# SCUT-CCNL/3DSIFT

Measured on AMD Instinct MI355X. Metric: Mvoxels/s end-to-end KpSiftAlgorithm on 512^3 fp32, higher is better.
Workload: dtype f32

## Files before the change

### 3dsift_amd/capi.py

```python
import ctypes as C
import os

import numpy as np

HERE = os.path.dirname(os.path.abspath(__file__))
LIB_PATH = os.environ.get("S3D_LIB") or os.path.join(HERE, "libsift3d_hip.so")
DESC = 768

KP_DTYPE = np.dtype(
    [
        ("x", "<f4"), ("y", "<f4"), ("z", "<f4"),
        ("scale", "<f4"),
        ("octave", "<i4"), ("level", "<i4"),
        ("rx", "<f4"), ("ry", "<f4"), ("rz", "<f4"),
        ("win", "<f4", (3,)),
        ("eigvalue", "<f4", (3,)),
        ("eigvector", "<f4", (9,)),
        ("Rotation", "<f4", (9,)),
        ("str_tensor", "<f4", (9,)),
    ]
)
assert KP_DTYPE.itemsize == 168

SYMBOLS = [
# ... 5 lines not shown
    "sift3d_match_handles",
    "sift3d_default_detect_options", "sift3d_set_detect_options", "sift3d_get_detect_options", "sift3d_get_refined",
    "sift3d_default_ransac_options", "sift3d_fit_affine", "sift3d_fit_affine_local",
    "sift3d_default_icgn_options", "sift3d_icgn_init_from_fits", "sift3d_icgn",
    "sift3d_device_count", "sift3d_error_string", "sift3d_last_error",
    "sift3d_slab_min_halo", "sift3d_slab_arena_floats", "sift3d_slab_create", "sift3d_slab_buffer", "sift3d_slab_upload",
    "sift3d_slab_input_absmax", "sift3d_slab_input_scale", "sift3d_slab_level", "sift3d_slab_level_hw", "sift3d_slab_halo_planes",
    "sift3d_slab_sync", "sift3d_slab_get_dogmax", "sift3d_slab_set_dogmax", "sift3d_slab_detect", "sift3d_slab_describe",
    "sift3d_slab_decimate", "sift3d_slab_admits", "sift3d_slab_set_ghost", "sift3d_slab_min_halo_ghost", "sift3d_create_seeded", "sift3d_seed_upload", "sift3d_set_describe_partition",
    "sift3d_export_device", "sift3d_import_descriptors_device", "sift3d_run_partial_orientation",
    "sift3d_export_orientation_device", "sift3d_import_orientation_device", "sift3d_run_describe",
    "sift3d_set_stream", "sift3d_slab_export_dogmax_device", "sift3d_slab_import_dogmax_device", "sift3d_slab_decimate_async",
    "sift3d_slab_set_desc_partial", "sift3d_slab_min_halo_partial", "sift3d_slab_record_bytes", "sift3d_slab_desc_reach", "sift3d_slab_orient",
    "sift3d_slab_export_records", "sift3d_slab_describe_partial", "sift3d_slab_describe_finish", "sift3d_slab_orient_launch",
    "sift3d_slab_orient_count",
    "sift3d_slab_keypoints_launch", "sift3d_slab_keypoints_count", "sift3d_slab_describe_finish_launch", "sift3d_slab_describe_finish_count",
    "sift3d_seed_buffer", "sift3d_sharded_plan", "sift3d_slab_describe_launch", "sift3d_sharded_traffic",
    "sift3d_sharded_create", "sift3d_sharded_create_ex", "sift3d_sharded_run", "sift3d_sharded_num_keypoints", "sift3d_sharded_get_keypoints", "sift3d_sharded_info",
    "sift3d_sharded_error", "sift3d_sharded_destroy",
    "sift3d_test_hook", "sift3d_debug_counters", "sift3d_debug_face_lookup", "sift3d_match_times", "sift3d_debug_copy_bandwidth",
    "sift3d_match_warmup", "sift3d_test_staging_slice", "sift3d_test_slab_plan", "sift3d_test_sharded_time_rank",
]
HOOKS = {"dog_eager": 0, "glast_eager": 1, "det_serial": 2, "separable": 3, "desc_nocache": 4, "match_nodma": 5, "one_stream": 6,
         "desc_mass_shift": 7, "list_cap": 8, "peer_copy": 9, "desc_nosplit": 10, "march_tiles": 11, "desc_exact_cells": 12, "lazy_generic": 13, "sharded_fail_rank": 14}
ORIENT_WORDS = 34
SHARDED_PARTIAL_WINDOWS = 1
SHARDED_WHOLE_WINDOWS = 2
SHARDED_COPY_TRANSPORT = 4
SHARDED_GHOST_OCTAVE0 = 8


class Params(C.Structure):
    _fields_ = [("num_kp_levels", C.c_int), ("sigma_default", C.c_float), ("sigma_n_default", C.c_float),
                ("peak_thresh", C.c_float), ("max_eig_thres", C.c_float), ("corner_thresh", C.c_float)]


class DetectOptions(C.Structure):
    _fields_ = [("neighbours", C.c_int), ("refine", C.c_int), ("max_offset", C.c_float), ("contrast_thresh", C.c_float),
                ("edge_ratio", C.c_float), ("reserved", C.c_int * 3)]


assert C.sizeof(DetectOptions) == 32

REFINED_DTYPE = np.dtype([("rx", "<f4"), ("ry", "<f4"), ("rz", "<f4"), ("scale", "<f4"), ("offset", "<f4", (4,)), ("contrast", "<f4")])
assert REFINED_DTYPE.itemsize == 36


# ... 919 lines not shown
```

### 3dsift_amd/csrc/context.hip

```cpp
#include <float.h>
#include <math.h>
#include <stdlib.h>
#include <string.h>

#include <algorithm>
#include <atomic>
#include <mutex>
#include <thread>

#include "ctx_internal.h"

#pragma clang fp contract(off)

namespace s3d {

static thread_local std::string g_last_error;
void set_last_error(const std::string &s) { g_last_error = s; }

int set_device(int device) {
	int n = 0;
	if (hipGetDeviceCount(&n) != hipSuccess || n <= 0) {
		set_last_error("no HIP device visible: this library has no CPU fallback");
		return SIFT3D_ERR_NO_DEVICE;
	}
// ... 25 lines not shown
	S3D_HIP(hipMalloc(&c->d_kpout, sizeof(sift3d_keypoint) * (size_t)c->kp_cap));
	S3D_HIP(hipMalloc(&c->d_desc, sizeof(float) * kDesc * (size_t)c->kp_cap));
	S3D_HIP(hipMalloc(&c->d_xyz, sizeof(float) * 3 * (size_t)c->kp_cap));
	{
		const unsigned scap = 4096;
		const size_t words = (size_t)scap * (kDesc + 8 + 1);
		int *base = nullptr;
		S3D_HIP(hipMalloc(&base, sizeof(int) * words));
		hipError_t me = hipMemsetAsync(base, 0, sizeof(int) * words, c->stream);
		if (me == hipSuccess) me = hipStreamSynchronize(c->stream);
		if (me != hipSuccess) {
			hipFree(base);
			set_last_error(std::string("HIP error: ") + hipGetErrorString(me) + " (clearing the split-window scratch)");
			return SIFT3D_ERR_HIP;
		}
		c->dsplit.gacc = base;
		c->dsplit.gmass = reinterpret_cast<float *>(base + (size_t)scap * kDesc);
		c->dsplit.gdone = reinterpret_cast<unsigned *>(base + (size_t)scap * (kDesc + 8));
		c->dsplit.cap = scap;
	}
	S3D_HIP(hipMalloc(&c->d_prov, sizeof(unsigned) * ((size_t)c->ext_cap + 1)));
	c->det.prov = c->d_prov; c->det.prov_count = c->d_prov + c->ext_cap; c->det.prov_cap = c->ext_cap;
	if (c->det_o.size() > 1) {
		const size_t n2 = c->det_o.size() - 1;
		const unsigned slice = std::max(64u, (unsigned)(c->ext_cap / n2));
		S3D_HIP(hipMalloc(&c->d_prov2, sizeof(unsigned) * ((size_t)slice + 1) * n2));
		for (size_t o = 1; o < c->det_o.size(); o++) {
			c->det_o[o].prov = c->d_prov2 + (o - 1) * ((size_t)slice + 1);
			c->det_o[o].prov_count = c->det_o[o].prov + slice;
			c->det_o[o].prov_cap = slice;
		}
	}
	return SIFT3D_OK;
}

extern "C" void sift3d_default_params(sift3d_params *p) {
	if (!p) return;
	p->num_kp_levels = 3;
	p->sigma_default = 1.6f;
	p->sigma_n_default = 1.15f;
	p->peak_thresh = 0.1f;
	p->max_eig_thres = 0.9f;
	p->corner_thresh = 0.4f;
}

extern "C" void sift3d_default_detect_options(sift3d_detect_options *o) {
	if (!o) return;
	memset(o, 0, sizeof(*o));
	o->neighbours = 8;
	o->refine = 0;
	o->max_offset = 0.5f;
	o->contrast_thresh = 0.0f;
// ... 525 lines not shown
		DetectOpts dopt;
		dopt.neighbours = c->dopt.neighbours; dopt.refine = c->dopt.refine;
		dopt.max_offset = c->dopt.max_offset; dopt.contrast_thresh = c->dopt.contrast_thresh; dopt.edge_ratio = c->dopt.edge_ratio;
		const DetectOpts *dop = c->run_full ? &dopt : nullptr;
		if (upto >= 3)
			for (int o = 0; o < c->noct; o++) {
				DetectLevels &DL = DLs[(size_t)o];
				memset(&DL, 0, sizeof(DL));
				for (int i = 1; i <= nl; i++) {
					DL.cur[i - 1] = c->dog[(size_t)o * c->nd + i].d;
					DL.prev[i - 1] = c->dog[(size_t)o * c->nd + i - 1].d;
					DL.next[i - 1] = c->dog[(size_t)o * c->nd + i + 1].d;
					DL.absmax_bits[i - 1] = c->d_dogmax + (size_t)o * c->nd + i;
					DL.level_id[i - 1] = i;
					DL.scale[i - 1] = c->dog[(size_t)o * c->nd + i].scale;
				}
				if (c->dog_elide) {
					DL.prev0_hi = c->gss[(size_t)o * c->ng + 1].d; DL.prev0_lo = c->gss[(size_t)o * c->ng].d;
					DL.nextl_hi = c->gss[(size_t)o * c->ng + c->nd].d; DL.nextl_lo = c->gss[(size_t)o * c->ng + c->nd - 1].d;
					DL.nextl_slot = nl - 1;
					if (c->g_last_elide) { DL.nextl_hi = nullptr; DL.lazy_src = DL.nextl_lo; }
				}
			}
		hipStream_t sb = two ? c->ostream[1] : st;
		if (early) {
			const Level &C0 = c->dog[(size_t)0 * c->nd + 1];
			S3D_HIP(hipEventRecord(c->ev_det_fork, st));
			launch_detect_mark(DLs[0], nl, C0.nx, C0.ny, C0.zr_all(), c->p.peak_thresh, 0 + c->octave_base, c->det, st, lt, dop);
			S3D_HIP(hipStreamWaitEvent(sb, c->ev_det_fork, 0));
			for (int o = 1; o < c->noct; o++) S3D_HIP(hipStreamWaitEvent(sb, c->ev_done[o], 0));
			S3D_HIP(hipEventRecord(c->ev[1], sb));
			S3D_HIP(hipEventRecord(c->ev[2], sb));
		} else {
			for (int o = 1; o < c->noct; o++) S3D_HIP(hipStreamWaitEvent(st, c->ev_done[o], 0));
			S3D_HIP(hipEventRecord(c->ev[1], st));
			S3D_HIP(hipEventRecord(c->ev[2], st));
		}
		if (upto >= 3) {
			if (two && !early) { S3D_HIP(hipEventRecord(c->ev_det_fork, st)); S3D_HIP(hipStreamWaitEvent(sb, c->ev_det_fork, 0)); }
			if (two) {
				hipStream_t sc = (c->noct > 2 && c->ostream.size() > 2 && c->ostream[2] != st && c->ostream[2] != sb) ? c->ostream[2] : sb;
				const bool own = early && sc != sb;
				if (sc != sb && !own) { S3D_HIP(hipEventRecord(c->ev_det_fork2, sb)); S3D_HIP(hipStreamWaitEvent(sc, c->ev_det_fork2, 0)); }
				for (int o = 1; o < c->noct; o++) {
					const Level &C = c->dog[(size_t)o * c->nd + 1];
					if (own && o >= 2) S3D_HIP(hipStreamWaitEvent(sc, c->ev_done[o], 0));
					launch_detect_mark(DLs[(size_t)o], nl, C.nx, C.ny, C.zr_all(), c->p.peak_thresh, o + c->octave_base, c->det_o[(size_t)o], o == 1 ? sb : sc, lt, dop);
				}
				S3D_HIP(hipEventRecord(c->ev_det_join, sb));
				if (sc != sb) { S3D_HIP(hipEventRecord(c->ev_det_join2, sc)); S3D_HIP(hipStreamWaitEvent(sb, c->ev_det_join2, 0)); S3D_HIP(hipEventRecord(c->ev_det_join, sb)); }
			}
			std::vector<DetectEmitItem> rest;
			for (int o = 0; o < c->noct; o++) {
				const Level &C = c->dog[(size_t)o * c->nd + 1];
				const DetectBufs &b = (two && o > 0) ? c->det_o[(size_t)o] : c->det;
				if (!(two && o > 0) && !(early && o == 0)) launch_detect_mark(DLs[(size_t)o], nl, C.nx, C.ny, C.zr_all(), c->p.peak_thresh, o + c->octave_base, b, st, lt, dop);
				if (two && o == 1) S3D_HIP(hipStreamWaitEvent(st, c->ev_det_join, 0));
				if (two && o > 0 && c->noct - 1 <= 8) rest.push_back(DetectEmitItem{&DLs[(size_t)o], nl, C.nx, C.ny, C.zr_all(), o + c->octave_base, &b});
				else launch_detect_emit(DLs[(size_t)o], nl, C.nx, C.ny, C.zr_all(), o + c->octave_base, b, c->d_ext, c->ext_cap, st);
			}
			if (!rest.empty()) launch_detect_emit_multi(rest.data(), (int)rest.size(), c->d_ext, c->ext_cap, c->d_total, st);
		}
		S3D_HIP(hipEventRecord(c->ev[3], st));
		if (upto >= 4) {
			launch_orient(c->d_ext, c->d_codes, c->d_total, c->ext_cap, c->d_levels, c->d_luts, c->d_lutpool, c->p.max_eig_thres,
			              c->p.corner_thresh, part_orient ? c->part_rank : 0, part_orient ? c->part_world : 1, c->d_order, c->d_nkp + 3, st);
			launch_slots(c->d_ext, c->d_codes, c->d_total, c->ext_cap, c->d_nkp, c->d_order, c->kp_cap, c->d_slots_part, st);
		}
		S3D_HIP(hipEventRecord(c->ev[4], st));
		if (upto >= 5) {
			launch_describe(c->d_ext, c->d_total, c->ext_cap, c->d_levels, c->d_luts, c->d_lutpool, c->d_desc, c->kp_cap, c->part_rank,
			                c->part_world, c->d_order, c->d_nkp, c->d_nkp + 1, st, c->desc_lut_lds, &c->dsplit);
		}
		if (upto >= 4) launch_finalize(c->d_ext, c->d_total, c->ext_cap, upto >= 5, c->d_kpout, c->d_xyz, c->kp_cap, st);
		if (upto >= 4 && c->run_refine) {
			DogTable T;
			memset(&T, 0, sizeof(T));
			T.octave_base = c->octave_base;
			for (int o = 0; o < c->noct && o < kDogTabOct; o++) {
				const Level &D0 = c->dog[(size_t)o * c->nd];
				T.nx[o] = D0.nx; T.ny[o] = D0.ny;
// ... 308 lines not shown
```

### 3dsift_amd/csrc/kernels_detect.hip

```cpp
#include <stdio.h>
#include <string.h>
#include <stdlib.h>

#include <algorithm>

#include "sift3d_internal.h"

namespace s3d {

#ifndef S3D_DET_ROWS
#define S3D_DET_ROWS 32
#endif
#ifndef S3D_DET_QUEUE
#define S3D_DET_QUEUE 640
#endif
#ifndef S3D_DETDIAG
#define S3D_DETDIAG 0
#endif
#ifndef S3D_DET_LEAN
#define S3D_DET_LEAN 1
#endif
#ifndef S3D_DET_XPRE
#define S3D_DET_XPRE 0
#endif
constexpr int kRows = S3D_DET_ROWS;
constexpr int kThreads = 256;

constexpr int kQueue = S3D_DET_QUEUE;
__global__ void __launch_bounds__(kThreads) k_mark(DetectLevels L, int nx, int ny, ZRange zr, int nyb, float peak_thresh,
                                                   unsigned long long *__restrict__ masks, unsigned *__restrict__ block_counts,
                                                   unsigned *__restrict__ prov, unsigned *__restrict__ prov_count, unsigned prov_cap,
                                                   unsigned *__restrict__ total) {
	__shared__ unsigned s_cnt[kThreads / 64];
	__shared__ uint2 s_q[kThreads / 64][kQueue];
	extern __shared__ unsigned long long s_mask_dyn[];
	const int segw = min((nx + 63) >> 6, 64);
	const int b = blockIdx.x;
	const int nz = zr.zo1 - zr.zo0;
	const int yb = b % nyb, zi = (b / nyb) % nz, lvl = b / (nyb * nz);
	const int z = zr.zo0 + zi;
	const int zg = z + zr.zoff;
	const float *__restrict__ cur = L.cur[lvl];
	const float *__restrict__ prev = L.prev[lvl];
	const float *__restrict__ next = L.next[lvl];
	const bool lazy_prev = lvl == 0 && L.prev0_hi != nullptr, lazy_next = lvl == L.nextl_slot && L.nextl_hi != nullptr;
	const bool lazy_g = lvl == L.nextl_slot && L.lazy_src != nullptr;
	const float thr = peak_thresh * __uint_as_float(*L.absmax_bits[lvl]);
	const int wpr = (nx + 63) >> 6;
	const int lane = threadIdx.x & 63, wid = threadIdx.x >> 6;
	const size_t sy = (size_t)nx, sz = (size_t)nx * ny;
	const bool z_in = (zg >= 1 && zg <= zr.nzg - 2);
	const int y0 = yb * kRows;
	constexpr int kBatch = 8;
	const int nrows = min(kRows, ny - y0);
	const int swid = __builtin_amdgcn_readfirstlane(wid);
	const int r_lo = swid * (kRows / 4), r_hi = min(nrows, (swid + 1) * (kRows / 4));
	uint2 *q = s_q[swid];
	unsigned long long *mloc = s_mask_dyn + (size_t)swid * (kRows / 4) * segw;
	for (int i = lane; i < (kRows / 4) * segw; i += 64) mloc[i] = 0ull;
	const unsigned long long lt = (1ull << lane) - 1ull;
// ... 139 lines not shown
					evaluate(qn, 64, seg0);
				}
			}
		}
		if (qn > 0) evaluate(0, qn, seg0);
		qn = 0;
		for (int ry = r_lo; ry < r_hi; ry++) {
			unsigned long long *mrow = masks + ((size_t)(lvl * nz + zi) * ny + (y0 + ry)) * wpr;
			for (int xw = seg0 + lane; xw < seg1; xw += 64) {
				const unsigned long long m = mloc[(ry - r_lo) * segw + xw - seg0];
				mrow[xw] = m;
				cnt += (unsigned)__popcll(m);
				mloc[(ry - r_lo) * segw + xw - seg0] = 0ull;
			}
		}
	}
#pragma unroll
	for (int o = 32; o > 0; o >>= 1) cnt += __shfl_xor(cnt, o, 64);
	if (lane == 0) s_cnt[wid] = cnt;
	__syncthreads();
	if (threadIdx.x == 0) block_counts[b] = s_cnt[0] + s_cnt[1] + s_cnt[2] + s_cnt[3];
}

__device__ __forceinline__ void lazy_tap_src(int p, int d, int n, int &lo, int &hi, float &frac, bool interior) {
	if (interior) { lo = hi = p - d; frac = 0.0f; return; }
	const int dim_end = n - 1;
	float c = (float)p - (float)d * 1.0f;
	if (c < 0.0f) c = -1.0f * c;
	else if (c >= (float)dim_end) c = (float)(2 * dim_end) - c - 0.1f;
	lo = (int)c;
	frac = c - (float)lo;
	hi = lo + 1;
	lo = min(max(lo, 0), dim_end);
	hi = min(max(hi, 0), dim_end);
}
static_assert(kLazySlots / 2 - 1 == 25, "k_lazy_next's wide instantiation covers kLazySlots");
constexpr int kLwN = 17, kLwPieces = kLwN * kLwN * 5, kLwInstr = (kLwPieces + 63) / 64, kLwFloats = kLwInstr * 256, kLwWaves = 2;
__global__ void __launch_bounds__(64 * kLwWaves) k_lazy_wave(DetectLevels L, Taps t, int nx, int ny, ZRange zr, int nyb,
                                                            const unsigned *__restrict__ prov, const unsigned *__restrict__ prov_count,
                                                            unsigned prov_cap, unsigned long long *__restrict__ masks,
                                                            unsigned *__restrict__ block_counts) {
	__shared__ __attribute__((aligned(1024))) float s_buf[kLwWaves][kLwFloats];
	constexpr int H = 8, N = kLwN;
	const int lane = threadIdx.x & 63, wid = __builtin_amdgcn_readfirstlane((int)(threadIdx.x >> 6));
	float *blk = s_buf[wid];
	const unsigned lds_base = (unsigned)(size_t)blk;
	const unsigned count = min(*prov_count, prov_cap);
	const int lvl = L.nextl_slot;
	const float *__restrict__ src = L.lazy_src;
	const float *__restrict__ cur = L.cur[lvl];
	const int wpr = (nx + 63) >> 6, nzs = zr.zo1 - zr.zo0, nzg = zr.nzg;
	const size_t sy = (size_t)nx, sz = (size_t)nx * ny;
	unsigned voff[kLwInstr];
#pragma unroll
	for (int j = 0; j < kLwInstr; j++) {
		const int p = min(64 * j + lane, kLwPieces - 1), row = p / 5, q = p - 5 * row, zi = row / N, yi = row - zi * N;
		voff[j] = (unsigned)(((size_t)zi * sz + (size_t)yi * sy + (size_t)(4 * q)) * sizeof(float));
	}
	const unsigned nwaves = gridDim.x * kLwWaves;
	for (unsigned e = blockIdx.x * kLwWaves + (unsigned)wid; e < count; e += nwaves) {
		const unsigned ent = prov[e];
		const size_t ic = (size_t)(ent & 0x7FFFFFFFu);
		const bool as_max = (ent >> 31) != 0;
		const int zl = (int)(ic / sz), rem = (int)(ic - (size_t)zl * sz), y = rem / nx, x = rem - y * nx;
		const int zg = zl + zr.zoff;
		if (!(x >= H && x <= nx - 2 - H && y >= H && y <= ny - 2 - H && zg >= H && zg <= nzg - 2 - H)) continue;
		const int shift = min(max(0, x + 11 - (nx - 1)), x - H);
		const float *base = src + ic - (size_t)H * sz - (size_t)H * sy - (size_t)(H + shift);
#pragma unroll
		for (int j = 0; j < kLwInstr; j++) {
			unsigned keep;
			asm volatile("s_mov_b32 %0, m0\n\ts_mov_b32 m0, %3\n\ts_nop 0\n\tglobal_load_lds_dwordx4 %1, %2\n\ts_mov_b32 m0, %0"
			             : "=&s"(keep) : "v"(voff[j]), "s"(base), "s"(lds_base + 1024u * (unsigned)j) : "memory");
		}
		const float centre = src[ic], v = cur[ic];
		asm volatile("s_waitcnt vmcnt(0)" ::: "memory");
		__builtin_amdgcn_wave_barrier();
#pragma unroll
		for (int rq = 0; rq < (N * N + 63) / 64; rq++) {
			const int row = min(lane + 64 * rq, N * N - 1);
			const float *r = blk + row * 20 + shift;
			float acc = 0.0f;
#pragma unroll
// ... 12 lines not shown
			__builtin_amdgcn_fence(__ATOMIC_RELEASE, "wavefront");
			__builtin_amdgcn_wave_barrier();
			if (lane < N) blk[pl * N * 20] = acc;
		}
		__builtin_amdgcn_fence(__ATOMIC_RELEASE, "wavefront");
		__builtin_amdgcn_wave_barrier();
		__builtin_amdgcn_fence(__ATOMIC_ACQUIRE, "wavefront");
		{
			float acc = 0.0f;
#pragma unroll
			for (int k = 0; k < N; k++) acc = acc + t.w[k] * blk[(2 * H - k) * N * 20];
			const float n7 = (acc - centre) * (-1.0f);
			if (lane == 0 && (as_max ? (v > n7) : (v < n7))) {
				const int zi = zl - zr.zo0;
				atomicOr(&masks[((size_t)(lvl * nzs + zi) * ny + y) * wpr + (x >> 6)], 1ull << (x & 63));
				atomicAdd(&block_counts[(lvl * nzs + zi) * nyb + y / kRows], 1u);
			}
		}
		__builtin_amdgcn_fence(__ATOMIC_RELEASE, "wavefront");
		__builtin_amdgcn_wave_barrier();
	}
}

template <int kLT>
__global__ void __launch_bounds__(256) k_lazy_next(DetectLevels L, Taps t, int nx, int ny, ZRange zr, int nyb,
                                                   const unsigned *__restrict__ prov, const unsigned *__restrict__ prov_count,
                                                   unsigned prov_cap, unsigned long long *__restrict__ masks,
                                                   unsigned *__restrict__ block_counts, int skip_interior) {
	constexpr int kLR = kLT + 1;
	constexpr int kLP = kLR + 1;
	__shared__ float s_blk[kLR * kLR * kLP];
	__shared__ float s_x[kLR * kLR];
	__shared__ float s_y[kLR];
	__shared__ float s_w[kMaxTaps];
	__shared__ int s_lo[3][kLT], s_hi[3][kLT];
	__shared__ float s_fr[3][kLT];
	__shared__ int s_rng[6];
	const int hw = t.hw, nt = 2 * hw + 1, tid = threadIdx.x;
	for (int i = tid; i < nt; i += 256) s_w[i] = t.w[i];
	const unsigned count = min(*prov_count, prov_cap);
	const int lvl = L.nextl_slot;
	const float *__restrict__ src = L.lazy_src;
	const float *__restrict__ cur = L.cur[lvl];
	const int wpr = (nx + 63) >> 6, nzs = zr.zo1 - zr.zo0, nzg = zr.nzg;
	const size_t sy = (size_t)nx, sz = (size_t)nx * ny;
	__shared__ unsigned s_list[256];
	__shared__ unsigned s_nlist;
	for (unsigned e0 = blockIdx.x; e0 < count; e0 += 256 * gridDim.x) {
	__syncthreads();
	if (tid == 0) s_nlist = 0u;
	__syncthreads();
	if (e0 + (unsigned)tid * gridDim.x < count) {
		const unsigned ent = prov[e0 + (unsigned)tid * gridDim.x];
		const size_t ic = (size_t)(ent & 0x7FFFFFFFu);
		const int zl = (int)(ic / sz), rem = (int)(ic - (size_t)zl * sz), y = rem / nx, x = rem - y * nx;
		const int zg = zl + zr.zoff;
		const bool inner = x >= hw && x <= nx - 2 - hw && y >= hw && y <= ny - 2 - hw && zg >= hw && zg <= nzg - 2 - hw;
		if (!(skip_interior && inner)) s_list[atomicAdd(&s_nlist, 1u)] = ent;
	}
	__syncthreads();
	const unsigned nlist = s_nlist;
	for (unsigned li = 0; li < nlist; li++) {
		const unsigned ent = s_list[li];
		const size_t ic = (size_t)(ent & 0x7FFFFFFFu);
		const bool as_max = (ent >> 31) != 0;
		const int zl = (int)(ic / sz), rem = (int)(ic - (size_t)zl * sz), y = rem / nx, x = rem - y * nx;
		const int zg = zl + zr.zoff;
		const bool ix = x >= hw && x <= nx - 2 - hw, iy = y >= hw && y <= ny - 2 - hw, iz = zg >= hw && zg <= nzg - 2 - hw;
		__syncthreads();
		if (tid < 3 * nt) {
			const int ax = tid / nt, k = tid - ax * nt;
			int lo, hi; float fr;
			if (ax == 0) lazy_tap_src(x, k - hw, nx, lo, hi, fr, ix);
			else if (ax == 1) lazy_tap_src(y, k - hw, ny, lo, hi, fr, iy);
			else lazy_tap_src(zg, k - hw, nzg, lo, hi, fr, iz);
			s_lo[ax][k] = lo; s_hi[ax][k] = hi; s_fr[ax][k] = fr;
// ... 56 lines not shown
		if (tid == 0) {
			const float *pl = s_y - zmin;
			float acc = 0.0f;
			if (iz) {
				for (int k = 0; k < nt; k++) acc = acc + s_w[k] * pl[s_lo[2][k]];
			} else {
				for (int k = 0; k < nt; k++) {
					const float f = s_fr[2][k];
					acc = acc + s_w[k] * ((1.0f - f) * pl[s_lo[2][k]] + f * pl[s_hi[2][k]]);
				}
			}
			const float n7 = (acc - src[ic]) * (-1.0f);
			const float v = cur[ic];
			if (as_max ? (v > n7) : (v < n7)) {
				const int zi = zl - zr.zo0;
				atomicOr(&masks[((size_t)(lvl * nzs + zi) * ny + y) * wpr + (x >> 6)], 1ull << (x & 63));
				atomicAdd(&block_counts[(lvl * nzs + zi) * nyb + y / kRows], 1u);
			}
		}
	}
	}
}

__device__ __forceinline__ unsigned scan_octave(const unsigned *__restrict__ block_counts, unsigned *__restrict__ block_offsets, unsigned nblocks,
                                                unsigned base, unsigned *s_wave) {
	const unsigned t = threadIdx.x;
	const unsigned chunk = (((nblocks + 1023u) / 1024u) + 3u) & ~3u;
	const unsigned lo = min(t * chunk, nblocks), hi = min(lo + chunk, nblocks);
	const bool vec = (((size_t)block_counts | (size_t)block_offsets) & 15) == 0 && hi - lo == chunk && chunk <= 32;
	unsigned cnt[32];
	unsigned sum = 0;
	if (vec) {
#pragma unroll
		for (unsigned q = 0; q < 8; q++)
			if (q * 4 < chunk) {
				const uint4 c4 = *reinterpret_cast<const uint4 *>(block_counts + lo + 4 * q);
				cnt[4 * q] = c4.x; cnt[4 * q + 1] = c4.y; cnt[4 * q + 2] = c4.z; cnt[4 * q + 3] = c4.w;
				sum += c4.x + c4.y + c4.z + c4.w;
			}
	} else {
		for (unsigned i = lo; i < hi; i++) sum += block_counts[i];
	}
	unsigned v = sum;
	const int lane = t & 63, wid = t >> 6;
#pragma unroll
	for (int o = 1; o < 64; o <<= 1) {
// ... 25 lines not shown
	__syncthreads();
	const unsigned nbase = s_wave[0];
	__syncthreads();
	return nbase;
}

__global__ void __launch_bounds__(1024) k_scan(const unsigned *__restrict__ block_counts, unsigned *__restrict__ block_offsets,
                                               unsigned nblocks, unsigned *__restrict__ total) {
	__shared__ unsigned s_wave[16];
	const unsigned nb = scan_octave(block_counts, block_offsets, nblocks, total[0], s_wave);
	if (threadIdx.x == 0) total[0] = nb;
}

struct EmitOct {
	const unsigned long long *masks;
	const unsigned *counts;
	unsigned *offsets;
	int nx, ny, nyb, octave;
	ZRange zr;
	unsigned nblocks, block0;
	int level_id[kMaxKpLevels];
	float scale[kMaxKpLevels];
};
struct EmitMulti { EmitOct o[8]; int n; };
__global__ void __launch_bounds__(1024) k_scan_multi(EmitMulti M, unsigned *__restrict__ total) {
	__shared__ unsigned s_wave[16];
	unsigned base = total[0];
	__syncthreads();
	for (int k = 0; k < M.n; k++) base = scan_octave(M.o[k].counts, M.o[k].offsets, M.o[k].nblocks, base, s_wave);
	if (threadIdx.x == 0) total[0] = base;
}

__device__ __forceinline__ void emit_block(int b, const unsigned long long *__restrict__ masks, const unsigned *__restrict__ block_offsets, int nx,
                                           int ny, const ZRange &zr, int nyb, int octave, const int *level_id, const float *scale,
                                           DevKp *__restrict__ out, unsigned cap, unsigned *__restrict__ total, unsigned *s_wave) {
	const int nz = zr.zo1 - zr.zo0;
	const int yb = b % nyb, zi = (b / nyb) % nz, lvl = b / (nyb * nz);
	const int z = zr.zo0 + zi + zr.zoff;
	const int wpr = (nx + 63) >> 6;
	const int y0 = yb * kRows;
	const int nwords = min(kRows, ny - y0) * wpr;
	const int lane = threadIdx.x & 63, wid = threadIdx.x >> 6;
	unsigned running = block_offsets[b];
	for (int w0 = 0; w0 < nwords; w0 += kThreads) {
		const int wi = w0 + threadIdx.x;
		unsigned long long m = 0;
		int y = 0, xw = 0;
// ... 34 lines not shown
			}
			pos++;
		}
		running += all;
	}
}

__global__ void __launch_bounds__(kThreads) k_emit(const unsigned long long *__restrict__ masks,
                                                   const unsigned *__restrict__ block_offsets, int nx, int ny, ZRange zr, int nyb,
                                                   int octave, DetectLevels L, DevKp *__restrict__ out, unsigned cap,
                                                   unsigned *__restrict__ total) {
	__shared__ unsigned s_wave[kThreads / 64];
	emit_block((int)blockIdx.x, masks, block_offsets, nx, ny, zr, nyb, octave, L.level_id, L.scale, out, cap, total, s_wave);
}

__global__ void __launch_bounds__(kThreads) k_emit_multi(EmitMulti M, DevKp *__restrict__ out, unsigned cap, unsigned *__restrict__ total) {
	__shared__ unsigned s_wave[kThreads / 64];
	int k = 0;
	while (k + 1 < M.n && blockIdx.x >= M.o[k + 1].block0) k++;
	const EmitOct &E = M.o[k];
	emit_block((int)(blockIdx.x - E.block0), E.masks, E.offsets, E.nx, E.ny, E.zr, E.nyb, E.octave, E.level_id, E.scale, out, cap, total, s_wave);
}

void launch_detect_mark(const DetectLevels &L, int nlevels, int nx, int ny, const ZRange &zr, float peak_thresh, int octave,
                        const DetectBufs &b, hipStream_t st, const Taps *lazy_taps, const DetectOpts *opt) {
	if (opt) { launch_mark_full(L, nlevels, nx, ny, zr, kRows, peak_thresh, *opt, b, st); return; }
	const int nyb = (ny + kRows - 1) / kRows;
	const int nzl = zr.zo1 - zr.zo0;
	if (nzl <= 0) return;
	const unsigned nblocks = (unsigned)(nlevels * nzl * nyb);
	if (nblocks == 0) return;
	const bool lazy = L.lazy_src != nullptr && lazy_taps != nullptr && b.prov != nullptr;
	if (lazy) (void)hipMemsetAsync(b.prov_count, 0, sizeof(unsigned), st);
	const size_t mask_lds = sizeof(unsigned long long) * (kThreads / 64) * (kRows / 4) * (size_t)std::min((nx + 63) >> 6, 64);
	hipLaunchKernelGGL(k_mark, dim3(nblocks), dim3(kThreads), mask_lds, st, L, nx, ny, zr, nyb, peak_thresh, b.masks, b.block_counts, b.prov,
	                   b.prov_count, b.prov_cap, b.total);
	if (lazy) {
		const bool wave_form = lazy_taps->hw == 8 && !hook(SIFT3D_HOOK_LAZY_GENERIC) && (size_t)nx * (size_t)ny * 17u * sizeof(float) < ((size_t)1 << 32);
		if (wave_form)
			hipLaunchKernelGGL(k_lazy_wave, dim3(256 * 3), dim3(64 * kLwWaves), 0, st, L, *lazy_taps, nx, ny, zr, nyb, b.prov, b.prov_count, b.prov_cap,
			                   b.masks, b.block_counts);
		if (2 * lazy_taps->hw + 1 <= 17)
			hipLaunchKernelGGL(k_lazy_next<17>, dim3(wave_form ? 1536 : 1024), dim3(256), 0, st, L, *lazy_taps, nx, ny, zr, nyb, b.prov, b.prov_count, b.prov_cap,
			                   b.masks, b.block_counts, wave_form ? 1 : 0);
		else
			hipLaunchKernelGGL(k_lazy_next<25>, dim3(512), dim3(256), 0, st, L, *lazy_taps, nx, ny, zr, nyb, b.prov, b.prov_count, b.prov_cap,
			                   b.masks, b.block_counts, 0);
	}
}

void launch_detect_emit(const DetectLevels &L, int nlevels, int nx, int ny, const ZRange &zr, int octave, const DetectBufs &b, DevKp *out,
                        unsigned cap, hipStream_t st) {
	const int nyb = (ny + kRows - 1) / kRows;
	const int nzl = zr.zo1 - zr.zo0;
	if (nzl <= 0) return;
	const unsigned nblocks = (unsigned)(nlevels * nzl * nyb);
	if (nblocks == 0) return;
	hipLaunchKernelGGL(k_scan, dim3(1), dim3(1024), 0, st, b.block_counts, b.block_offsets, nblocks, b.total);
	hipLaunchKernelGGL(k_emit, dim3(nblocks), dim3(kThreads), 0, st, b.masks, b.block_offsets, nx, ny, zr, nyb, octave, L, out, cap,
	                   b.total);
}

void launch_detect_emit_multi(const DetectEmitItem *items, int n, DevKp *out, unsigned cap, unsigned *total, hipStream_t st) {
	EmitMulti M;
	memset(&M, 0, sizeof(M));
	unsigned blocks = 0;
	for (int k = 0; k < n && M.n < 8; k++) {
		const DetectEmitItem &it = items[k];
		const int nyb = (it.ny + kRows - 1) / kRows, nzl = it.zr.zo1 - it.zr.zo0;
		if (nzl <= 0) continue;
		const unsigned nblocks = (unsigned)(it.nlevels * nzl * nyb);
		if (nblocks == 0) continue;
		EmitOct &E = M.o[M.n++];
		E.masks = it.b->masks; E.counts = it.b->block_counts; E.offsets = it.b->block_offsets;
		E.nx = it.nx; E.ny = it.ny; E.nyb = nyb; E.octave = it.octave; E.zr = it.zr; E.nblocks = nblocks; E.block0 = blocks;
		for (int l = 0; l < kMaxKpLevels; l++) { E.level_id[l] = it.L->level_id[l]; E.scale[l] = it.L->scale[l]; }
		blocks += nblocks;
	}
	if (M.n == 0) return;
	hipLaunchKernelGGL(k_scan_multi, dim3(1), dim3(1024), 0, st, M, total);
	hipLaunchKernelGGL(k_emit_multi, dim3(blocks), dim3(kThreads), 0, st, M, out, cap, total);
}

void launch_detect_octave(const DetectLevels &L, int nlevels, int nx, int ny, const ZRange &zr, float peak_thresh, int octave,
                          const DetectBufs &b, DevKp *out, unsigned cap, hipStream_t st, const Taps *lazy_taps) {
	launch_detect_mark(L, nlevels, nx, ny, zr, peak_thresh, octave, b, st, lazy_taps);
	launch_detect_emit(L, nlevels, nx, ny, zr, octave, b, out, cap, st);
}

void preload_detect_kernels() { hipFuncAttributes a; (void)hipFuncGetAttributes(&a, reinterpret_cast<const void *>(&k_scan)); }
// ... 3 lines not shown
```

### 3dsift_amd/csrc/sift3d_internal.h

```cpp
#pragma once

#include <hip/hip_runtime.h>
#include <stdint.h>

#include <string>
#include <vector>

#include "../../include/sift3d_hip.h"
#include "../../include/sift3d_hip_test.h"

#pragma clang fp contract(off)

namespace s3d {

#ifndef S3D_MAX_HW
#define S3D_MAX_HW 64
#endif
constexpr int kMaxHW = S3D_MAX_HW;
constexpr int kMaxTaps = 2 * kMaxHW + 1;
constexpr int kDesc = SIFT3D_DESC_NUMEL;
constexpr int kFaces = 20;

struct Taps {
	int hw;
// ... 115 lines not shown
	const unsigned *absmax_bits[kMaxKpLevels];
	int level_id[kMaxKpLevels];
	float scale[kMaxKpLevels];
};
constexpr int kLazySlots = 52;
struct DetectOpts {
	int neighbours = 8, refine = 0;
	float max_offset = 0.5f, contrast_thresh = 0.0f, edge_ratio = 0.0f;
};
void launch_detect_mark(const DetectLevels &L, int nlevels, int nx, int ny, const ZRange &zr, float peak_thresh, int octave,
                        const DetectBufs &b, hipStream_t st, const Taps *lazy_taps, const DetectOpts *opt = nullptr);
void launch_mark_full(const DetectLevels &L, int nlevels, int nx, int ny, const ZRange &zr, int rows, float peak_thresh, const DetectOpts &opt,
                      const DetectBufs &b, hipStream_t st);
constexpr int kDogTabOct = 12, kDogTabLv = 8;
struct DogTable {
	const float *d[kDogTabOct][kDogTabLv];
	int nx[kDogTabOct], ny[kDogTabOct];
	int octave_base;
};
void launch_detect_emit(const DetectLevels &L, int nlevels, int nx, int ny, const ZRange &zr, int octave, const DetectBufs &b, DevKp *out,
                        unsigned cap, hipStream_t st);
struct DetectEmitItem { const DetectLevels *L; int nlevels, nx, ny; ZRange zr; int octave; const DetectBufs *b; };
void launch_detect_emit_multi(const DetectEmitItem *items, int n, DevKp *out, unsigned cap, unsigned *total, hipStream_t st);
void launch_detect_octave(const DetectLevels &L, int nlevels, int nx, int ny, const ZRange &zr, float peak_thresh, int octave,
                          const DetectBufs &b, DevKp *out, unsigned cap, hipStream_t st, const Taps *lazy_taps = nullptr);

#ifdef __HIPCC__
typedef const float __attribute__((address_space(1))) *gfloat_p;
__device__ __forceinline__ gfloat_p as_global(const float *p) { return (gfloat_p)p; }
#endif

struct LevelRef {
	const float *d;
	int nx, ny, nz;
	float unit;
	int zoff;
};
void launch_orient(DevKp *kps, int *codes, const unsigned *d_count, unsigned cap, const LevelRef *d_levels ,
                   const WinLut *d_luts, const float *d_lutpool, float max_eig, float corner, int part_rank, int part_world,
                   int *redo_list , unsigned *redo_count,
                   hipStream_t st);
constexpr int kOrientWords = 34;
void launch_orient_pack(const DevKp *kps, const unsigned *d_count, unsigned cap, int *dst, int part_rank, int part_world, hipStream_t st);
void launch_orient_unpack(DevKp *kps, int *codes, const unsigned *d_count, unsigned cap, const int *src, hipStream_t st);
size_t slots_scratch_words();
void launch_slots(DevKp *kps, const int *codes, const unsigned *d_count, unsigned cap, unsigned *d_nkp, int *order, unsigned kp_cap,
// ... 89 lines not shown
```

Measured before the change: 19410.

## Batch small-octave detect marking and lazy refinement into multi-octave launches

Octaves 2 and up, which are small, no longer get separate mark and lazy-refinement launches. They are grouped into one table-driven k_mark launch plus combined lazy wave and next launches, with the grids split by each octave's voxel share. The prov_count counters are packed contiguously so one memset clears them all. Octave 0 is also folded into the multi-octave emit pass. The aim is to cut kernel launch and memset overhead on tiny grids, at the cost of a larger kernel-argument struct and a per-block search through the table.

```diff
diff --git a/3dsift_amd/capi.py b/3dsift_amd/capi.py
--- a/3dsift_amd/capi.py
+++ b/3dsift_amd/capi.py
@@ -51,7 +51,8 @@
     "sift3d_match_warmup", "sift3d_test_staging_slice", "sift3d_test_slab_plan", "sift3d_test_sharded_time_rank",
 ]
 HOOKS = {"dog_eager": 0, "glast_eager": 1, "det_serial": 2, "separable": 3, "desc_nocache": 4, "match_nodma": 5, "one_stream": 6,
-         "desc_mass_shift": 7, "list_cap": 8, "peer_copy": 9, "desc_nosplit": 10, "march_tiles": 11, "desc_exact_cells": 12, "lazy_generic": 13, "sharded_fail_rank": 14}
+         "desc_mass_shift": 7, "list_cap": 8, "peer_copy": 9, "desc_nosplit": 10, "march_tiles": 11, "desc_exact_cells": 12, "lazy_generic": 13, "sharded_fail_rank": 14,
+         "det_unbatched": 15}
 ORIENT_WORDS = 34
 SHARDED_PARTIAL_WINDOWS = 1
 SHARDED_WHOLE_WINDOWS = 2
diff --git a/3dsift_amd/csrc/context.hip b/3dsift_amd/csrc/context.hip
--- a/3dsift_amd/csrc/context.hip
+++ b/3dsift_amd/csrc/context.hip
@@ -71,12 +71,12 @@
 	S3D_HIP(hipMalloc(&c->d_prov, sizeof(unsigned) * ((size_t)c->ext_cap + 1)));
 	c->det.prov = c->d_prov; c->det.prov_count = c->d_prov + c->ext_cap; c->det.prov_cap = c->ext_cap;
 	if (c->det_o.size() > 1) {
-		const size_t n2 = c->det_o.size() - 1;
+		const size_t n2 = c->det_o.size() - 1, head = (n2 + 63) & ~(size_t)63;
 		const unsigned slice = std::max(64u, (unsigned)(c->ext_cap / n2));
-		S3D_HIP(hipMalloc(&c->d_prov2, sizeof(unsigned) * ((size_t)slice + 1) * n2));
+		S3D_HIP(hipMalloc(&c->d_prov2, sizeof(unsigned) * (head + (size_t)slice * n2)));
 		for (size_t o = 1; o < c->det_o.size(); o++) {
-			c->det_o[o].prov = c->d_prov2 + (o - 1) * ((size_t)slice + 1);
-			c->det_o[o].prov_count = c->det_o[o].prov + slice;
+			c->det_o[o].prov = c->d_prov2 + head + (o - 1) * (size_t)slice;
+			c->det_o[o].prov_count = c->d_prov2 + (o - 1);
 			c->det_o[o].prov_cap = slice;
 		}
 	}
@@ -648,11 +648,20 @@
 					if (c->g_last_elide) { DL.nextl_hi = nullptr; DL.lazy_src = DL.nextl_lo; }
 				}
 			}
+		const bool tables_fit = c->noct - 1 <= 8 && !hook(SIFT3D_HOOK_DET_UNBATCHED);
+		static const int det_batch_mode = dev_tune_i("S3D_DET_BATCH", 1), emit_one_mode = dev_tune_i("S3D_EMIT_ONE", 1);
+		const bool batch = two && tables_fit && !dop && det_batch_mode != 0 && c->noct - 2 <= detect_mark_multi_max();
+		const bool emit_one = tables_fit && emit_one_mode != 0;
+		static const int lazy_all_mode = dev_tune_i("S3D_LAZY_ALL", 0);
+		const bool lazy_all = batch && early && lt != nullptr && lazy_all_mode != 0 && c->noct <= detect_mark_multi_max();
 		hipStream_t sb = two ? c->ostream[1] : st;
 		if (early) {
 			const Level &C0 = c->dog[(size_t)0 * c->nd + 1];
 			S3D_HIP(hipEventRecord(c->ev_det_fork, st));
-			launch_detect_mark(DLs[0], nl, C0.nx, C0.ny, C0.zr_all(), c->p.peak_thresh, 0 + c->octave_base, c->det, st, lt, dop);
+			if (lazy_all) {
+				const DetectEmitItem i0{&DLs[0], nl, C0.nx, C0.ny, C0.zr_all(), 0 + c->octave_base, &c->det};
+				launch_detect_mark_multi(&i0, 1, c->p.peak_thresh, st, lt, 1);
+			} else launch_detect_mark(DLs[0], nl, C0.nx, C0.ny, C0.zr_all(), c->p.peak_thresh, 0 + c->octave_base, c->det, st, lt, dop);
 			S3D_HIP(hipStreamWaitEvent(sb, c->ev_det_fork, 0));
 			for (int o = 1; o < c->noct; o++) S3D_HIP(hipStreamWaitEvent(sb, c->ev_done[o], 0));
 			S3D_HIP(hipEventRecord(c->ev[1], sb));
@@ -668,11 +677,17 @@
 				hipStream_t sc = (c->noct > 2 && c->ostream.size() > 2 && c->ostream[2] != st && c->ostream[2] != sb) ? c->ostream[2] : sb;
 				const bool own = early && sc != sb;
 				if (sc != sb && !own) { S3D_HIP(hipEventRecord(c->ev_det_fork2, sb)); S3D_HIP(hipStreamWaitEvent(sc, c->ev_det_fork2, 0)); }
+				std::vector<DetectEmitItem> small;
 				for (int o = 1; o < c->noct; o++) {
 					const Level &C = c->dog[(size_t)o * c->nd + 1];
 					if (own && o >= 2) S3D_HIP(hipStreamWaitEvent(sc, c->ev_done[o], 0));
-					launch_detect_mark(DLs[(size_t)o], nl, C.nx, C.ny, C.zr_all(), c->p.peak_thresh, o + c->octave_base, c->det_o[(size_t)o], o == 1 ? sb : sc, lt, dop);
+					if (batch && o >= 2) small.push_back(DetectEmitItem{&DLs[(size_t)o], nl, C.nx, C.ny, C.zr_all(), o + c->octave_base, &c->det_o[(size_t)o]});
+					else if (lazy_all) {
+						const DetectEmitItem i1{&DLs[(size_t)o], nl, C.nx, C.ny, C.zr_all(), o + c->octave_base, &c->det_o[(size_t)o]};
+						launch_detect_mark_multi(&i1, 1, c->p.peak_thresh, sb, lt, 1);
+					} else launch_detect_mark(DLs[(size_t)o], nl, C.nx, C.ny, C.zr_all(), c->p.peak_thresh, o + c->octave_base, c->det_o[(size_t)o], o == 1 ? sb : sc, lt, dop);
 				}
+				if (!small.empty()) launch_detect_mark_multi(small.data(), (int)small.size(), c->p.peak_thresh, sc, lt, lazy_all ? 1 : 3);
 				S3D_HIP(hipEventRecord(c->ev_det_join, sb));
 				if (sc != sb) { S3D_HIP(hipEventRecord(c->ev_det_join2, sc)); S3D_HIP(hipStreamWaitEvent(sb, c->ev_det_join2, 0)); S3D_HIP(hipEventRecord(c->ev_det_join, sb)); }
 			}
@@ -682,7 +697,15 @@
 				const DetectBufs &b = (two && o > 0) ? c->det_o[(size_t)o] : c->det;
 				if (!(two && o > 0) && !(early && o == 0)) launch_detect_mark(DLs[(size_t)o], nl, C.nx, C.ny, C.zr_all(), c->p.peak_thresh, o + c->octave_base, b, st, lt, dop);
 				if (two && o == 1) S3D_HIP(hipStreamWaitEvent(st, c->ev_det_join, 0));
-				if (two && o > 0 && c->noct - 1 <= 8) rest.push_back(DetectEmitItem{&DLs[(size_t)o], nl, C.nx, C.ny, C.zr_all(), o + c->octave_base, &b});
+				if (lazy_all && o == 1) {
+					std::vector<DetectEmitItem> all;
+					for (int q = 0; q < c->noct; q++) {
+						const Level &Cq = c->dog[(size_t)q * c->nd + 1];
+						all.push_back(DetectEmitItem{&DLs[(size_t)q], nl, Cq.nx, Cq.ny, Cq.zr_all(), q + c->octave_base, q ? &c->det_o[(size_t)q] : &c->det});
+					}
+					launch_detect_mark_multi(all.data(), (int)all.size(), c->p.peak_thresh, st, lt, 2);
+				}
+				if (two && (o > 0 || emit_one) && tables_fit) rest.push_back(DetectEmitItem{&DLs[(size_t)o], nl, C.nx, C.ny, C.zr_all(), o + c->octave_base, &b});
 				else launch_detect_emit(DLs[(size_t)o], nl, C.nx, C.ny, C.zr_all(), o + c->octave_base, b, c->d_ext, c->ext_cap, st);
 			}
 			if (!rest.empty()) launch_detect_emit_multi(rest.data(), (int)rest.size(), c->d_ext, c->ext_cap, c->d_total, st);
diff --git a/3dsift_amd/csrc/kernels_detect.hip b/3dsift_amd/csrc/kernels_detect.hip
--- a/3dsift_amd/csrc/kernels_detect.hip
+++ b/3dsift_amd/csrc/kernels_detect.hip
@@ -27,15 +27,37 @@
 constexpr int kThreads = 256;
 
 constexpr int kQueue = S3D_DET_QUEUE;
-__global__ void __launch_bounds__(kThreads) k_mark(DetectLevels L, int nx, int ny, ZRange zr, int nyb, float peak_thresh,
-                                                   unsigned long long *__restrict__ masks, unsigned *__restrict__ block_counts,
-                                                   unsigned *__restrict__ prov, unsigned *__restrict__ prov_count, unsigned prov_cap,
-                                                   unsigned *__restrict__ total) {
+constexpr int kMarkMax = 8;
+struct MarkOct {
+	DetectLevels L;
+	int nx, ny, nyb, skip_interior;
+	ZRange zr;
+	unsigned long long *masks;
+	unsigned *block_counts, *prov, *prov_count, *total;
+	unsigned prov_cap;
+	unsigned block0;
+	unsigned wave0, wave_n;
+	unsigned next0, next_n;
+};
+template <int kN> struct MarkTable { MarkOct o[kN]; int n; };
+typedef MarkTable<kMarkMax> MarkMulti;
+
+template <int kN>
+__global__ void __launch_bounds__(kThreads) k_mark(MarkTable<kN> M, float peak_thresh) {
+	int k = 0;
+	if (kN > 1) while (k + 1 < M.n && blockIdx.x >= M.o[k + 1].block0) k++;
+	const MarkOct &E = M.o[k];
+	const DetectLevels &L = E.L;
+	const int b = (int)(blockIdx.x - (kN > 1 ? E.block0 : 0u));
+	const int nx = E.nx, ny = E.ny, nyb = E.nyb;
+	const ZRange &zr = E.zr;
+	unsigned long long *__restrict__ masks = E.masks;
+	unsigned *__restrict__ block_counts = E.block_counts, *__restrict__ prov = E.prov, *__restrict__ prov_count = E.prov_count, *__restrict__ total = E.total;
+	const unsigned prov_cap = E.prov_cap;
 	__shared__ unsigned s_cnt[kThreads / 64];
 	__shared__ uint2 s_q[kThreads / 64][kQueue];
 	extern __shared__ unsigned long long s_mask_dyn[];
 	const int segw = min((nx + 63) >> 6, 64);
-	const int b = blockIdx.x;
 	const int nz = zr.zo1 - zr.zo0;
 	const int yb = b % nyb, zi = (b / nyb) % nz, lvl = b / (nyb * nz);
 	const int z = zr.zo0 + zi;
@@ -221,6 +243,7 @@
 	if (threadIdx.x == 0) block_counts[b] = s_cnt[0] + s_cnt[1] + s_cnt[2] + s_cnt[3];
 }
 
+
 __device__ __forceinline__ void lazy_tap_src(int p, int d, int n, int &lo, int &hi, float &frac, bool interior) {
 	if (interior) { lo = hi = p - d; frac = 0.0f; return; }
 	const int dim_end = n - 1;
@@ -235,10 +258,10 @@
 }
 static_assert(kLazySlots / 2 - 1 == 25, "k_lazy_next's wide instantiation covers kLazySlots");
 constexpr int kLwN = 17, kLwPieces = kLwN * kLwN * 5, kLwInstr = (kLwPieces + 63) / 64, kLwFloats = kLwInstr * 256, kLwWaves = 2;
-__global__ void __launch_bounds__(64 * kLwWaves) k_lazy_wave(DetectLevels L, Taps t, int nx, int ny, ZRange zr, int nyb,
-                                                            const unsigned *__restrict__ prov, const unsigned *__restrict__ prov_count,
-                                                            unsigned prov_cap, unsigned long long *__restrict__ masks,
-                                                            unsigned *__restrict__ block_counts) {
+__device__ __forceinline__ void lazy_wave_body(const DetectLevels &L, const Taps &t, int nx, int ny, const ZRange &zr, int nyb,
+                                               const unsigned *__restrict__ prov, const unsigned *__restrict__ prov_count,
+                                               unsigned prov_cap, unsigned long long *__restrict__ masks,
+                                               unsigned *__restrict__ block_counts, const unsigned wg, const unsigned nwg) {
 	__shared__ __attribute__((aligned(1024))) float s_buf[kLwWaves][kLwFloats];
 	constexpr int H = 8, N = kLwN;
 	const int lane = threadIdx.x & 63, wid = __builtin_amdgcn_readfirstlane((int)(threadIdx.x >> 6));
@@ -256,8 +279,8 @@
 		const int p = min(64 * j + lane, kLwPieces - 1), row = p / 5, q = p - 5 * row, zi = row / N, yi = row - zi * N;
 		voff[j] = (unsigned)(((size_t)zi * sz + (size_t)yi * sy + (size_t)(4 * q)) * sizeof(float));
 	}
-	const unsigned nwaves = gridDim.x * kLwWaves;
-	for (unsigned e = blockIdx.x * kLwWaves + (unsigned)wid; e < count; e += nwaves) {
+	const unsigned nwaves = nwg * kLwWaves;
+	for (unsigned e = wg * kLwWaves + (unsigned)wid; e < count; e += nwaves) {
 		const unsigned ent = prov[e];
 		const size_t ic = (size_t)(ent & 0x7FFFFFFFu);
 		const bool as_max = (ent >> 31) != 0;
@@ -316,11 +339,25 @@
 	}
 }
 
+__global__ void __launch_bounds__(64 * kLwWaves) k_lazy_wave(DetectLevels L, Taps t, int nx, int ny, ZRange zr, int nyb,
+                                                            const unsigned *__restrict__ prov, const unsigned *__restrict__ prov_count,
+                                                            unsigned prov_cap, unsigned long long *__restrict__ masks,
+                                                            unsigned *__restrict__ block_counts) {
+	lazy_wave_body(L, t, nx, ny, zr, nyb, prov, prov_count, prov_cap, masks, block_counts, blockIdx.x, gridDim.x);
+}
+
+__global__ void __launch_bounds__(64 * kLwWaves) k_lazy_wave_multi(MarkMulti M, Taps t) {
+	int k = 0;
+	while (k + 1 < M.n && blockIdx.x >= M.o[k + 1].wave0) k++;
+	const MarkOct &E = M.o[k];
+	lazy_wave_body(E.L, t, E.nx, E.ny, E.zr, E.nyb, E.prov, E.prov_count, E.prov_cap, E.masks, E.block_counts, blockIdx.x - E.wave0, E.wave_n);
+}
+
 template <int kLT>
-__global__ void __launch_bounds__(256) k_lazy_next(DetectLevels L, Taps t, int nx, int ny, ZRange zr, int nyb,
-                                                   const unsigned *__restrict__ prov, const unsigned *__restrict__ prov_count,
-                                                   unsigned prov_cap, unsigned long long *__restrict__ masks,
-                                                   unsigned *__restrict__ block_counts, int skip_interior) {
+__device__ __forceinline__ void lazy_next_body(const DetectLevels &L, const Taps &t, int nx, int ny, const ZRange &zr, int nyb,
+                                               const unsigned *__restrict__ prov, const unsigned *__restrict__ prov_count,
+                                               unsigned prov_cap, unsigned long long *__restrict__ masks,
+                                               unsigned *__restrict__ block_counts, int skip_interior, const unsigned wg, const unsigned nwg) {
 	constexpr int kLR = kLT + 1;
 	constexpr int kLP = kLR + 1;
 	__shared__ float s_blk[kLR * kLR * kLP];
@@ -340,12 +377,12 @@
 	const size_t sy = (size_t)nx, sz = (size_t)nx * ny;
 	__shared__ unsigned s_list[256];
 	__shared__ unsigned s_nlist;
-	for (unsigned e0 = blockIdx.x; e0 < count; e0 += 256 * gridDim.x) {
+	for (unsigned e0 = wg; e0 < count; e0 += 256 * nwg) {
 	__syncthreads();
 	if (tid == 0) s_nlist = 0u;
 	__syncthreads();
-	if (e0 + (unsigned)tid * gridDim.x < count) {
-		const unsigned ent = prov[e0 + (unsigned)tid * gridDim.x];
+	if (e0 + (unsigned)tid * nwg < count) {
+		const unsigned ent = prov[e0 + (unsigned)tid * nwg];
 		const size_t ic = (size_t)(ent & 0x7FFFFFFFu);
 		const int zl = (int)(ic / sz), rem = (int)(ic - (size_t)zl * sz), y = rem / nx, x = rem - y * nx;
 		const int zg = zl + zr.zoff;
@@ -448,6 +485,23 @@
 	}
 }
 
+template <int kLT>
+__global__ void __launch_bounds__(256) k_lazy_next(DetectLevels L, Taps t, int nx, int ny, ZRange zr, int nyb,
+                                                   const unsigned *__restrict__ prov, const unsigned *__restrict__ prov_count,
+                                                   unsigned prov_cap, unsigned long long *__restrict__ masks,
+                                                   unsigned *__restrict__ block_counts, int skip_interior) {
+	lazy_next_body<kLT>(L, t, nx, ny, zr, nyb, prov, prov_count, prov_cap, masks, block_counts, skip_interior, blockIdx.x, gridDim.x);
+}
+
+template <int kLT>
+__global__ void __launch_bounds__(256) k_lazy_next_multi(MarkMulti M, Taps t) {
+	int k = 0;
+	while (k + 1 < M.n && blockIdx.x >= M.o[k + 1].next0) k++;
+	const MarkOct &E = M.o[k];
+	lazy_next_body<kLT>(E.L, t, E.nx, E.ny, E.zr, E.nyb, E.prov, E.prov_count, E.prov_cap, E.masks, E.block_counts, E.skip_interior,
+	                    blockIdx.x - E.next0, E.next_n);
+}
+
 __device__ __forceinline__ unsigned scan_octave(const unsigned *__restrict__ block_counts, unsigned *__restrict__ block_offsets, unsigned nblocks,
                                                 unsigned base, unsigned *s_wave) {
 	const unsigned t = threadIdx.x;
@@ -519,7 +573,8 @@
 	int level_id[kMaxKpLevels];
 	float scale[kMaxKpLevels];
 };
-struct EmitMulti { EmitOct o[8]; int n; };
+constexpr int kEmitMax = 9;
+struct EmitMulti { EmitOct o[kEmitMax]; int n; };
 __global__ void __launch_bounds__(1024) k_scan_multi(EmitMulti M, unsigned *__restrict__ total) {
 	__shared__ unsigned s_wave[16];
 	unsigned base = total[0];
@@ -600,6 +655,10 @@
 	emit_block((int)(blockIdx.x - E.block0), E.masks, E.offsets, E.nx, E.ny, E.zr, E.nyb, E.octave, E.level_id, E.scale, out, cap, total, s_wave);
 }
 
+static bool lazy_wave_form(const Taps &t, int nx, int ny) {
+	return t.hw == 8 && !hook(SIFT3D_HOOK_LAZY_GENERIC) && (size_t)nx * (size_t)ny * 17u * sizeof(float) < ((size_t)1 << 32);
+}
+
 void launch_detect_mark(const DetectLevels &L, int nlevels, int nx, int ny, const ZRange &zr, float peak_thresh, int octave,
                         const DetectBufs &b, hipStream_t st, const Taps *lazy_taps, const DetectOpts *opt) {
 	if (opt) { launch_mark_full(L, nlevels, nx, ny, zr, kRows, peak_thresh, *opt, b, st); return; }
@@ -611,10 +670,13 @@
 	const bool lazy = L.lazy_src != nullptr && lazy_taps != nullptr && b.prov != nullptr;
 	if (lazy) (void)hipMemsetAsync(b.prov_count, 0, sizeof(unsigned), st);
 	const size_t mask_lds = sizeof(unsigned long long) * (kThreads / 64) * (kRows / 4) * (size_t)std::min((nx + 63) >> 6, 64);
-	hipLaunchKernelGGL(k_mark, dim3(nblocks), dim3(kThreads), mask_lds, st, L, nx, ny, zr, nyb, peak_thresh, b.masks, b.block_counts, b.prov,
-	                   b.prov_count, b.prov_cap, b.total);
+	MarkTable<1> M1;
+	memset(&M1, 0, sizeof(M1));
+	M1.n = 1; M1.o[0].L = L; M1.o[0].nx = nx; M1.o[0].ny = ny; M1.o[0].nyb = nyb; M1.o[0].zr = zr; M1.o[0].masks = b.masks; M1.o[0].block_counts = b.block_counts;
+	M1.o[0].prov = b.prov; M1.o[0].prov_count = b.prov_count; M1.o[0].total = b.total; M1.o[0].prov_cap = b.prov_cap;
+	hipLaunchKernelGGL(k_mark<1>, dim3(nblocks), dim3(kThreads), mask_lds, st, M1, peak_thresh);
 	if (lazy) {
-		const bool wave_form = lazy_taps->hw == 8 && !hook(SIFT3D_HOOK_LAZY_GENERIC) && (size_t)nx * (size_t)ny * 17u * sizeof(float) < ((size_t)1 << 32);
+		const bool wave_form = lazy_wave_form(*lazy_taps, nx, ny);
 		if (wave_form)
 			hipLaunchKernelGGL(k_lazy_wave, dim3(256 * 3), dim3(64 * kLwWaves), 0, st, L, *lazy_taps, nx, ny, zr, nyb, b.prov, b.prov_count, b.prov_cap,
 			                   b.masks, b.block_counts);
@@ -625,6 +687,63 @@
 			hipLaunchKernelGGL(k_lazy_next<25>, dim3(512), dim3(256), 0, st, L, *lazy_taps, nx, ny, zr, nyb, b.prov, b.prov_count, b.prov_cap,
 			                   b.masks, b.block_counts, 0);
 	}
+}
+
+int detect_mark_multi_max() { return kMarkMax; }
+void launch_detect_mark_multi(const DetectEmitItem *items, int n, float peak_thresh, hipStream_t st, const Taps *lazy_taps, int phases) {
+	MarkMulti M;
+	memset(&M, 0, sizeof(M));
+	unsigned blocks = 0;
+	int max_nx = 0;
+	double vox[kMarkMax], vox_sum = 0.0;
+	bool lazy = lazy_taps != nullptr, any_wave = false;
+	for (int k = 0; k < n && M.n < kMarkMax; k++) {
+		const DetectEmitItem &it = items[k];
+		const int nyb = (it.ny + kRows - 1) / kRows, nzl = it.zr.zo1 - it.zr.zo0;
+		if (nzl <= 0) continue;
+		const unsigned nblocks = (unsigned)(it.nlevels * nzl * nyb);
+		if (nblocks == 0) continue;
+		lazy = lazy && it.L->lazy_src != nullptr && it.b->prov != nullptr;
+		MarkOct &E = M.o[M.n];
+		E.L = *it.L;
+		E.nx = it.nx; E.ny = it.ny; E.nyb = nyb; E.zr = it.zr;
+		E.masks = it.b->masks; E.block_counts = it.b->block_counts; E.prov = it.b->prov; E.prov_count = it.b->prov_count; E.total = it.b->total;
+		E.prov_cap = it.b->prov_cap;
+		E.block0 = blocks;
+		blocks += nblocks;
+		max_nx = std::max(max_nx, it.nx);
+		vox[M.n] = (double)it.nx * it.ny * nzl;
+		vox_sum += vox[M.n];
+		M.n++;
+	}
+	if (M.n == 0) return;
+	if (phases & 1) {
+		if (lazy) {
+			bool packed = true;
+			for (int k = 1; k < M.n; k++) packed = packed && M.o[k].prov_count == M.o[0].prov_count + k;
+			if (packed) (void)hipMemsetAsync(M.o[0].prov_count, 0, sizeof(unsigned) * (size_t)M.n, st);
+			else for (int k = 0; k < M.n; k++) (void)hipMemsetAsync(M.o[k].prov_count, 0, sizeof(unsigned), st);
+		}
+		const size_t mask_lds = sizeof(unsigned long long) * (kThreads / 64) * (kRows / 4) * (size_t)std::min((max_nx + 63) >> 6, 64);
+		hipLaunchKernelGGL(k_mark<kMarkMax>, dim3(blocks), dim3(kThreads), mask_lds, st, M, peak_thresh);
+	}
+	if (!(phases & 2) || !lazy) return;
+	const bool narrow = 2 * lazy_taps->hw + 1 <= 17;
+	for (int k = 0; k < M.n; k++) any_wave = any_wave || lazy_wave_form(*lazy_taps, M.o[k].nx, M.o[k].ny);
+	const unsigned wave_grid = 256 * 3, next_grid = narrow ? (any_wave ? 1536u : 1024u) : 512u;
+	unsigned wave_blocks = 0, next_blocks = 0;
+	for (int k = 0; k < M.n; k++) {
+		MarkOct &E = M.o[k];
+		const bool wf = lazy_wave_form(*lazy_taps, E.nx, E.ny);
+		const double share = vox[k] / vox_sum;
+		E.skip_interior = wf ? 1 : 0;
+		E.wave0 = wave_blocks; E.wave_n = wf ? std::max(1u, (unsigned)(share * wave_grid)) : 0u;
+		E.next0 = next_blocks; E.next_n = std::max(1u, (unsigned)(share * next_grid));
+		wave_blocks += E.wave_n; next_blocks += E.next_n;
+	}
+	if (wave_blocks) hipLaunchKernelGGL(k_lazy_wave_multi, dim3(wave_blocks), dim3(64 * kLwWaves), 0, st, M, *lazy_taps);
+	if (narrow) hipLaunchKernelGGL(k_lazy_next_multi<17>, dim3(next_blocks), dim3(256), 0, st, M, *lazy_taps);
+	else hipLaunchKernelGGL(k_lazy_next_multi<25>, dim3(next_blocks), dim3(256), 0, st, M, *lazy_taps);
 }
 
 void launch_detect_emit(const DetectLevels &L, int nlevels, int nx, int ny, const ZRange &zr, int octave, const DetectBufs &b, DevKp *out,
@@ -643,7 +762,7 @@
 	EmitMulti M;
 	memset(&M, 0, sizeof(M));
 	unsigned blocks = 0;
-	for (int k = 0; k < n && M.n < 8; k++) {
+	for (int k = 0; k < n && M.n < kEmitMax; k++) {
 		const DetectEmitItem &it = items[k];
 		const int nyb = (it.ny + kRows - 1) / kRows, nzl = it.zr.zo1 - it.zr.zo0;
 		if (nzl <= 0) continue;
diff --git a/3dsift_amd/csrc/sift3d_internal.h b/3dsift_amd/csrc/sift3d_internal.h
--- a/3dsift_amd/csrc/sift3d_internal.h
+++ b/3dsift_amd/csrc/sift3d_internal.h
@@ -161,6 +161,8 @@
                         unsigned cap, hipStream_t st);
 struct DetectEmitItem { const DetectLevels *L; int nlevels, nx, ny; ZRange zr; int octave; const DetectBufs *b; };
 void launch_detect_emit_multi(const DetectEmitItem *items, int n, DevKp *out, unsigned cap, unsigned *total, hipStream_t st);
+int detect_mark_multi_max();
+void launch_detect_mark_multi(const DetectEmitItem *items, int n, float peak_thresh, hipStream_t st, const Taps *lazy_taps, int phases = 3);
 void launch_detect_octave(const DetectLevels &L, int nlevels, int nx, int ny, const ZRange &zr, float peak_thresh, int octave,
                           const DetectBufs &b, DevKp *out, unsigned cap, hipStream_t st, const Taps *lazy_taps = nullptr);
 
```

Result: no change. 19560 (median of 6 runs) (+0.8%).
